# pangfumin/badslam

Hardware: AMD Instinct MI355X
Metric: surfel x keyframe residual evaluations per second, full alternating BA iteration (higher is better)
Workload: dtype f32

## Files before the change

### badslam_amd/abi.py

```python
import ctypes as C

BSLAM_INVALID_DEPTH_BIT = 1 << 15
BSLAM_UNKNOWN_DEPTH = 65535
BSLAM_SURFEL_ACTIVE_FLAG = 1

SURFEL_X, SURFEL_Y, SURFEL_Z, SURFEL_NORMAL = 0, 1, 2, 3
SURFEL_RADIUS_SQUARED, SURFEL_COLOR, SURFEL_DESCRIPTOR1, SURFEL_DESCRIPTOR2 = 4, 5, 6, 7
SURFEL_ACCUM0 = 8
SURFEL_DATA_ATTRIBUTE_COUNT = 8
SURFEL_ATTRIBUTE_COUNT = 17

KF_ACTIVE, KF_COVISIBLE_ACTIVE, KF_INACTIVE = 0, 1, 2

TEX_FIXED_POINT_1_8 = 0
TEX_EXACT_FLOAT = 1

INVALID_INDEX = 0xFFFFFFFF


class Buffer2D(C.Structure):
    _fields_ = [("address", C.c_void_p), ("height", C.c_int32), ("width", C.c_int32), ("pitch", C.c_size_t)]


class Mat3x4(C.Structure):
# ... 138 lines not shown
    "bslam_compute_cost_and_residual_count_from_images": (C.c_int, [C.c_void_p, C.c_void_p, C.c_int, C.c_int, P(Camera4f), P(Camera4f), C.c_float,
                                                                   C.c_float, P(Buffer2D), P(Buffer2D), P(Buffer2D), P(Mat3x4), P(Buffer2D),
                                                                   P(Buffer2D), P(Buffer2D), P(C.c_uint32), P(C.c_float)]),
    "bslam_accumulate_pose_coeffs_from_images_gradmag": (C.c_int, [C.c_void_p, C.c_void_p, C.c_int, C.c_int, P(Camera4f), P(Camera4f), C.c_float, C.c_float,
                                                                  P(Buffer2D), P(Buffer2D), P(Buffer2D), P(Mat3x4), P(Buffer2D), P(Buffer2D), P(Buffer2D),
                                                                  P(C.c_uint32), P(C.c_float), P(C.c_float)]),
    "bslam_compute_cost_and_residual_count_from_images_gradmag": (C.c_int, [C.c_void_p, C.c_void_p, C.c_int, C.c_int, P(Camera4f), P(Camera4f), C.c_float,
                                                                           C.c_float, P(Buffer2D), P(Buffer2D), P(Buffer2D), P(Mat3x4), P(Buffer2D),
                                                                           P(Buffer2D), P(Buffer2D), P(C.c_uint32), P(C.c_float)]),
    "bslam_accumulate_pose_coeffs_from_images_batched": (C.c_int, [C.c_void_p, C.c_void_p, C.c_int, C.c_int, P(Camera4f), P(Camera4f), C.c_float,
                                                                  C.c_float, C.c_int, P(Buffer2D), P(Buffer2D), P(Buffer2D), P(Mat3x4), P(Buffer2D),
                                                                  P(Buffer2D), P(Buffer2D), P(C.c_uint32), P(C.c_float), P(C.c_float)]),
    "bslam_compute_sobel_gradient_magnitude": (C.c_int, [C.c_void_p, C.c_void_p, P(Buffer2D), P(Buffer2D)]),
    "bslam_calibrate_and_downsample_images": (C.c_int, [C.c_void_p, C.c_void_p, C.c_int, P(DepthParams), P(Buffer2D), P(Buffer2D), P(Buffer2D), P(Buffer2D),
                                                       P(Buffer2D), P(Buffer2D)]),
    "bslam_compact_surfels": (C.c_int, [C.c_void_p, C.c_void_p, C.c_uint32, P(C.c_uint32), P(Buffer2D), P(Buffer2D)]),
    "bslam_invalidate_keyframe_cache": (C.c_int, [C.c_void_p]),
    "bslam_comm_get_unique_id": (C.c_int, [C.c_void_p, C.c_size_t]),
    "bslam_comm_init": (C.c_int, [C.c_void_p, C.c_void_p, C.c_int, C.c_int]),
    "bslam_comm_destroy": (C.c_int, [C.c_void_p]),
    "bslam_comm_query": (C.c_int, [C.c_void_p, P(C.c_int), P(C.c_int)]),
    "bslam_set_culling": (C.c_int, [C.c_void_p, C.c_int]),
    "bslam_set_pose_keyframe_list": (C.c_int, [C.c_void_p, C.c_int]),
    "bslam_debug_cull_stats": (C.c_int, [C.c_void_p, P(C.c_uint64), P(C.c_uint64)]),
    "bslam_profile_enable": (C.c_int, [C.c_void_p, C.c_int]),
    "bslam_profile_read": (C.c_int, [C.c_void_p, C.c_int, P(C.c_int32), P(C.c_float)]),
    "bslam_profile_read_counters": (C.c_int, [C.c_void_p, P(C.c_uint64)]),
    "bslam_set_geometry_keyframe_chunk": (C.c_int, [C.c_void_p, C.c_int]),
    "bslam_assign_colors": (C.c_int, [C.c_void_p, C.c_void_p, _CAM, _CAM, _DP, C.c_int, _KFS, C.c_uint32, _BUF]),
    "bslam_debug_decode_normals": (C.c_int, [C.c_void_p, C.c_void_p, P(C.c_float)]),
    "bslam_debug_jacobians": (C.c_int, [C.c_void_p, C.c_void_p, C.c_int, C.c_int, P(C.c_float), P(C.c_float)]),
    "bslam_debug_wave_column_sums": (C.c_int, [C.c_void_p, C.c_void_p, C.c_int, C.c_int, C.POINTER(C.c_float), C.POINTER(C.c_float)]),
    "bslam_debug_desc_pair": (C.c_int, [C.c_void_p, C.c_void_p, C.c_int, P(C.c_float), P(C.c_float)]),
    "bslam_debug_quad_samples": (C.c_int, [C.c_void_p, C.c_void_p, C.c_int, C.c_int, C.c_int, C.c_int, P(C.c_uint8), C.c_int, P(C.c_float), C.c_int,
                                           P(C.c_float), P(C.c_uint16)]),
    "bslam_debug_count_pairs": (C.c_int, [
        C.c_void_p, C.c_void_p, _CAM, _DP, C.c_int, _KFS, C.c_uint32, _BUF, P(C.c_uint64), P(C.c_uint64)]),
    "bslam_accumulate_pose_estimation_coeffs": (C.c_int, [
        C.c_void_p, C.c_void_p, C.c_int, C.c_int, _CAM, _CAM, _DP, _BUF, _BUF, _BUF, P(Mat3x4),
        C.c_uint32, _BUF, C.c_int, P(C.c_uint32), P(C.c_float), P(C.c_float), P(C.c_float)]),
    "bslam_estimate_frame_poses_batched": (C.c_int, [
        C.c_void_p, C.c_void_p, C.c_int, C.c_int, _CAM, _CAM, _DP, C.c_int, _KFS,
        C.c_uint32, _BUF, C.c_int, P(SE3f), P(C.c_int32), P(C.c_int32), ALLREDUCE_FN, C.c_void_p]),
    "bslam_compute_ba_cost": (C.c_int, [
        C.c_void_p, C.c_void_p, C.c_int, C.c_int, _CAM, _CAM, _DP, C.c_int, _KFS,
        C.c_uint32, _BUF, _BUF, P(C.c_float), P(C.c_uint32), ALLREDUCE_FN, C.c_void_p]),
# ... 31 lines not shown
```

### badslam_amd/csrc/badslam_hip.hip

```cpp
#include <hip/hip_runtime.h>
#include <dlfcn.h>
#include <rocprim/device/device_radix_sort.hpp>

#include <algorithm>
#include <climits>
#include <cmath>
#include <cstdlib>
#include <cstring>
#include <initializer_list>
#include <new>

#include "context.hpp"
#include "geometry_kernels.hpp"
#include "intrinsics_kernels.hpp"
#include "pcg_kernels.hpp"
#include "lifecycle_kernels.hpp"
#include "preprocess_kernels.hpp"
#include "rectify_kernels.hpp"
#include "render_kernels.hpp"
#include "fusion_kernels.hpp"
#include "mesh_kernels.hpp"
#include "distance_kernels.hpp"
#include "registration_kernels.hpp"
#include "sampling_kernels.hpp"
#include "simplify_kernels.hpp"
#include "decimate_kernels.hpp"
#include "smooth_kernels.hpp"
#include "raycast_kernels.hpp"
#include "render_mesh_kernels.hpp"
#include "place_kernels.hpp"
#include "odometry_kernels.hpp"
#include "pose_kernels.hpp"
#include "cost_kernels.hpp"
// ... 421 lines not shown
  if (chunks < 1) chunks = 1;
  if (chunks > kf_count) chunks = kf_count;
  int per_block = (kf_count + chunks - 1) / chunks;
#ifndef BSLAM_POSE_MAX_KFS_PER_BLOCK
#define BSLAM_POSE_MAX_KFS_PER_BLOCK 0
#endif
  const int cap = BSLAM_POSE_MAX_KFS_PER_BLOCK > 0 ? BSLAM_POSE_MAX_KFS_PER_BLOCK : (tiles >= 8192 ? 64 : 32);
  per_block = (per_block + multiple - 1) / multiple * multiple;
  if (per_block > cap) per_block = cap;
  return per_block;
}

static unsigned long long* cull_stats_ptr(bslam_context* ctx) {
  return ctx->profiling ? (unsigned long long*)((uint8_t*)ctx->misc.ptr + kMiscCullStats) : nullptr;
}

struct PoseGrid {
  Schedule sc;
  int per_block;
  unsigned chunks;
  unsigned launch_chunks;
  dim3 grid;
};
static int plan_pose_grid(bslam_context* ctx, const Schedule& prepared, int kf_count, int multiple, int list_bound, PoseGrid* g) {
  g->sc = prepared;
#ifndef BSLAM_POSE_CULL_MIN_KEYFRAMES
#define BSLAM_POSE_CULL_MIN_KEYFRAMES 64
#endif
  if (kf_count < BSLAM_POSE_CULL_MIN_KEYFRAMES) g->sc.bounds = nullptr;
  g->per_block = choose_kfs_per_block((int)g->sc.slots, kf_count, multiple);
  g->chunks = (unsigned)((kf_count + g->per_block - 1) / g->per_block);
  g->launch_chunks = list_bound >= 0 ? (unsigned)std::max(1, (std::min(list_bound, kf_count) + g->per_block - 1) / g->per_block) : g->chunks;
  g->grid = dim3(8u * g->sc.slots_per_xcd * g->launch_chunks);
  return ctx->vis.reserve((size_t)g->chunks * g->sc.slots * sizeof(VisWord));
}

static int launch_pose_accumulate(bslam_context* ctx, hipStream_t stream, int use_depth, int use_desc, const CamConsts& c,
                                  int kf_count, uint32_t surfels_size, const bslam_buffer2d* surfels, const PoseState* states,
                                  int* tiles_out, bool reduce_rows = true, const SurfelWork* work = nullptr, int* kfs_per_block_out = nullptr,
                                  bool want_cost = false, const int* kf_list = nullptr, int kf_list_bound = 0) {
  SurfelWork local;
  int rc = BSLAM_OK;
  if (!work) {
    if ((rc = prepare_surfels(ctx, stream, surfels, surfels_size, pose_surfels_per_thread(use_desc != 0, surfels_size), kf_count, &local, use_desc != 0))) return rc;
    work = &local;
  }
  const int tiles = (int)work->sc.slots;
  *tiles_out = tiles;
  const int rows_per_kf = tiles;
  rc = ctx->partials.reserve((size_t)rows_per_kf * kf_count * kRow * sizeof(float));
  if (rc) return rc;
  rc = ctx->coeffs.reserve((size_t)kf_count * kRow * sizeof(float));
  if (rc) return rc;
#ifndef BSLAM_POSE_DESC_KF_MULTIPLE
#define BSLAM_POSE_DESC_KF_MULTIPLE 4
#endif
  PoseGrid g;
  if ((rc = plan_pose_grid(ctx, work->sc, kf_count, use_desc ? BSLAM_POSE_DESC_KF_MULTIPLE : 1, kf_list ? kf_list_bound : -1, &g))) return rc;
  const Schedule& sc = g.sc;
  const int per_block = g.per_block;
  if (kfs_per_block_out) *kfs_per_block_out = per_block;
  VisWord* vis = (VisWord*)ctx->vis.ptr;
  const dim3 grid = g.grid;
  const SurfelRows rows = work->rows;
  const KfDev* kfs = (const KfDev*)ctx->kf_table.ptr;
  float* partials = (float*)ctx->partials.ptr;
  static const unsigned debug_lds = getenv("BSLAM_DEBUG_POSE_LDS") ? (unsigned)atoi(getenv("BSLAM_DEBUG_POSE_LDS")) : 0u;
  {
  ProfScope prof(ctx, stream);
  const bool cost = want_cost;
#define BSLAM_LAUNCH_POSE(DEPTH, DESC, R)                                                                                                        \
  do {                                                                                                                                           \
    if (cost) hipLaunchKernelGGL((pose_accumulate_kernel<DEPTH, DESC, R, true>), grid, dim3(kPoseThreads), debug_lds, stream, c, kfs, kf_count, per_block, sc, rows, partials, rows_per_kf, states, vis, kf_list);  \
    else hipLaunchKernelGGL((pose_accumulate_kernel<DEPTH, DESC, R, false>), grid, dim3(kPoseThreads), debug_lds, stream, c, kfs, kf_count, per_block, sc, rows, partials, rows_per_kf, states, vis, kf_list); \
  } while (0)
  if (use_depth && use_desc) BSLAM_LAUNCH_POSE(true, true, kPoseRDesc);
  else if (use_depth && pose_surfels_per_thread(false, surfels_size) == kPoseRGeoLarge) BSLAM_LAUNCH_POSE(true, false, kPoseRGeoLarge);
  else if (use_depth) BSLAM_LAUNCH_POSE(true, false, kPoseRGeo);
  else BSLAM_LAUNCH_POSE(false, true, kPoseRDesc);
#undef BSLAM_LAUNCH_POSE
  }
  BSLAM_HIP_TRY(hipGetLastError());
  if (!reduce_rows) return BSLAM_OK;
  hipLaunchKernelGGL(pose_reduce_rows_kernel, dim3((unsigned)kf_count), dim3(1024), (unsigned)visit_map_bytes(tiles), stream, (const float*)partials, rows_per_kf, kf_count,
                     (float*)ctx->coeffs.ptr, states, (const VisWord*)vis, per_block, cull_stats_ptr(ctx), kf_list ? kf_list + 1 + kf_count : nullptr);
// ... 177 lines not shown
}

int bslam_set_xcd_schedule(bslam_context* ctx, int enable) {
  if (!ctx) return fail(BSLAM_ERR_INVALID_ARGUMENT, "context is null");
  ctx->use_schedule = enable != 0;
  ctx->order_key.clear();
  ctx->perm_key.clear();
  return BSLAM_OK;
}

int bslam_set_culling(bslam_context* ctx, int enable) {
  if (!ctx) return fail(BSLAM_ERR_INVALID_ARGUMENT, "context is null");
  ctx->culling = enable != 0;
  return BSLAM_OK;
}

int bslam_set_pose_keyframe_list(bslam_context* ctx, int min_keyframes) {
  if (!ctx) return fail(BSLAM_ERR_INVALID_ARGUMENT, "null context");
  if (min_keyframes < 0) return fail(BSLAM_ERR_INVALID_ARGUMENT, "min_keyframes must be >= 0");
  ctx->pose_list_min_keyframes = min_keyframes;
  return BSLAM_OK;
}

int bslam_debug_cull_stats(bslam_context* ctx, uint64_t* tested, uint64_t* culled) {
  if (!ctx) return fail(BSLAM_ERR_INVALID_ARGUMENT, "context is null");
  BSLAM_HIP_TRY(hipSetDevice(ctx->device));
  BSLAM_HIP_TRY(hipDeviceSynchronize());
  unsigned long long h[2] = {0, 0};
  BSLAM_HIP_TRY(hipMemcpy(h, (uint8_t*)ctx->misc.ptr + kMiscCullStats, sizeof(h), hipMemcpyDeviceToHost));
  BSLAM_HIP_TRY(hipMemset((uint8_t*)ctx->misc.ptr + kMiscCullStats, 0, sizeof(h)));
  if (tested) *tested = h[0];
  if (culled) *culled = h[0] - h[1];
  return BSLAM_OK;
}

int bslam_profile_enable(bslam_context* ctx, int enable) {
  if (!ctx) return fail(BSLAM_ERR_INVALID_ARGUMENT, "context is null");
  ctx->profiling = enable != 0;
  for (auto& ev : ctx->prof_pending) ctx->prof_pool.push_back(std::make_pair(ev.start, ev.stop));
  ctx->prof_pending.clear();
  for (int t = 0; t < 8; ++t) { ctx->prof_launches[t] = 0; ctx->prof_ms[t] = 0.f; }
  for (int i = 0; i < 8; ++i) ctx->prof_counter_base[i] = 0;
  if (ctx->prof_counters.ptr && ctx->prof_counter_slots) {
    BSLAM_HIP_TRY(hipSetDevice(ctx->device));
    BSLAM_HIP_TRY(hipDeviceSynchronize());
    BSLAM_HIP_TRY(hipMemset(ctx->prof_counters.ptr, 0, ctx->prof_counter_slots * sizeof(unsigned long long)));
// ... 282 lines not shown
  if (rc) return rc;
  std::vector<PoseState> states((size_t)keyframe_count);
  for (int k = 0; k < keyframe_count; ++k) {
    PoseState& st = states[k];
    std::memset(&st, 0, sizeof(st));
    std::memcpy(st.q, poses[k].q, sizeof(float) * 4);
    std::memcpy(st.t, poses[k].t, sizeof(float) * 3);
    st.converged = (keyframes[k].activation == BSLAM_KF_INACTIVE) ? 1 : 0;
  }
  const size_t state_bytes = states.size() * sizeof(PoseState);
  if ((rc = ctx->pose_state.reserve(state_bytes))) return rc;
  if ((rc = ctx->staging2.reserve(state_bytes + 64))) return rc;
  {
    void* stage = nullptr;
    if ((rc = ctx->upload_ring.acquire(state_bytes, &stage))) return rc;
    std::memcpy(stage, states.data(), state_bytes);
    BSLAM_HIP_TRY(hipMemcpyAsync(ctx->pose_state.ptr, stage, state_bytes, hipMemcpyHostToDevice, stream));
    if ((rc = ctx->upload_ring.commit(stream))) return rc;
  }

  PoseState* d_states = (PoseState*)ctx->pose_state.ptr;
  int* d_active = (int*)((uint8_t*)ctx->misc.ptr + kMiscActive);
  int* h_active = (int*)((uint8_t*)ctx->staging2.ptr + state_bytes);
  for (hipEvent_t& e : ctx->iter_done)
    if (!e) BSLAM_HIP_TRY(hipEventCreateWithFlags(&e, hipEventDisableTiming));
  for (hipEvent_t& e : ctx->solve_done)
    if (!e) BSLAM_HIP_TRY(hipEventCreateWithFlags(&e, hipEventDisableTiming));
  if (!ctx->copy_stream) BSLAM_HIP_TRY(hipStreamCreateWithFlags(&ctx->copy_stream, hipStreamNonBlocking));
  ctx->kf_table_host_ptr = nullptr;
  hipLaunchKernelGGL(pose_init_kernel, dim3((unsigned)((keyframe_count + 63) / 64)), dim3(64), 0, stream, keyframe_count,
                     (const PoseState*)d_states, (KfDev*)ctx->kf_table.ptr, d_active);
  BSLAM_HIP_TRY(hipGetLastError());

  SurfelWork work;
  if (surfels_size > 0 && (rc = prepare_surfels(ctx, stream, surfels, surfels_size, pose_surfels_per_thread(use_descriptor_residuals != 0, surfels_size), keyframe_count, &work, use_descriptor_residuals != 0))) return rc;

  int* d_list = nullptr;
  if (surfels_size > 0 && ctx->pose_list_min_keyframes > 0 && keyframe_count >= ctx->pose_list_min_keyframes) {
    if ((rc = ctx->pose_list.reserve((size_t)(1 + 2 * keyframe_count) * sizeof(int)))) return rc;
    d_list = (int*)ctx->pose_list.ptr;
    hipLaunchKernelGGL(pose_active_list_kernel, dim3(1), dim3(kActiveListThreads), 0, stream, keyframe_count, (const PoseState*)d_states, d_list);
    BSLAM_HIP_TRY(hipGetLastError());
  }
  int known_active = keyframe_count;

  auto enqueue_iteration = [&](int it) -> int {
    const int slot = it & 3;
    const bool exchange = allreduce != nullptr || has_exchange(ctx);
    const bool fused = surfels_size > 0 && !exchange;
    if (fused) {
      int tiles = 0, per_block = 1;
      int r = launch_pose_accumulate(ctx, stream, use_depth_residuals, use_descriptor_residuals, c, keyframe_count, surfels_size, surfels, d_states, &tiles, false, &work, &per_block,
                                     false, d_list, known_active);
      if (r) return r;
      {
        ProfScope prof(ctx, stream, BSLAM_PROF_POSE_REDUCE);
        hipLaunchKernelGGL(pose_reduce_solve_kernel, dim3((unsigned)keyframe_count), dim3(kReduceSolveThreads), (unsigned)visit_map_bytes(tiles), stream, (const float*)ctx->partials.ptr,
                           tiles, keyframe_count, d_states, (KfDev*)ctx->kf_table.ptr, d_active + slot, d_active + ((it + 1) & 3),
                           (const VisWord*)ctx->vis.ptr, per_block, cull_stats_ptr(ctx), d_list ? d_list + 1 + keyframe_count : nullptr);
      }
      BSLAM_HIP_TRY(hipGetLastError());
    } else {
      if (surfels_size > 0) {
        int tiles = 0;
        int r = launch_pose_accumulate(ctx, stream, use_depth_residuals, use_descriptor_residuals, c, keyframe_count, surfels_size, surfels, d_states, &tiles, true, &work, nullptr,
                                       false, d_list, known_active);
        if (r) return r;
      } else {
        int r = ctx->coeffs.reserve((size_t)keyframe_count * kRow * sizeof(float));
        if (r) return r;
        BSLAM_HIP_TRY(hipMemsetAsync(ctx->coeffs.ptr, 0, (size_t)keyframe_count * kRow * sizeof(float), stream));
      }
      {
        ProfScope prof(ctx, stream, BSLAM_PROF_EXCHANGE);
        if (allreduce) {
          const int arc = allreduce(allreduce_user, ctx->coeffs.ptr, (size_t)keyframe_count * kRow, stream);
          if (arc) return fail(BSLAM_ERR_HIP, "allreduce callback failed with %d", arc);
        } else if (exchange) {
          const int arc = exchange_sum(ctx, stream, (float*)ctx->coeffs.ptr, (size_t)keyframe_count * kRow);
          if (arc) return arc;
        }
      }
      hipLaunchKernelGGL(pose_solve_kernel, dim3((unsigned)((keyframe_count + 63) / 64)), dim3(64), 0, stream,
                         (const float*)ctx->coeffs.ptr, keyframe_count, d_states, (KfDev*)ctx->kf_table.ptr, d_active + slot, d_active + ((it + 1) & 3));
      BSLAM_HIP_TRY(hipGetLastError());
    }
    BSLAM_HIP_TRY(hipEventRecord(ctx->solve_done[slot], stream));
    BSLAM_HIP_TRY(hipStreamWaitEvent(ctx->copy_stream, ctx->solve_done[slot], 0));
    BSLAM_HIP_TRY(hipMemcpyAsync(h_active + slot, d_active + slot, sizeof(int), hipMemcpyDeviceToHost, ctx->copy_stream));
    BSLAM_HIP_TRY(hipEventRecord(ctx->iter_done[slot], ctx->copy_stream));
    if (d_list) {
      hipLaunchKernelGGL(pose_active_list_kernel, dim3(1), dim3(kActiveListThreads), 0, stream, keyframe_count, (const PoseState*)d_states, d_list);
      BSLAM_HIP_TRY(hipGetLastError());
    }
    return BSLAM_OK;
  };
  if (max_iterations > 0 && (rc = enqueue_iteration(0))) return rc;
  for (int it = 0; it < max_iterations; ++it) {
    if (it + 1 < max_iterations && (rc = enqueue_iteration(it + 1))) return rc;
    BSLAM_HIP_TRY(hipEventSynchronize(ctx->iter_done[it & 3]));
    if (h_active[it & 3] == 0) break;
    known_active = std::min(known_active, h_active[it & 3]);
  }
  BSLAM_HIP_TRY(hipMemcpyAsync(ctx->staging2.ptr, d_states, state_bytes, hipMemcpyDeviceToHost, stream));
  BSLAM_HIP_TRY(hipStreamSynchronize(stream));
  BSLAM_HIP_TRY(hipStreamSynchronize(ctx->copy_stream));
  const PoseState* out = (const PoseState*)ctx->staging2.ptr;
  for (int k = 0; k < keyframe_count; ++k) {
    std::memcpy(poses[k].q, out[k].q, sizeof(float) * 4);
    std::memcpy(poses[k].t, out[k].t, sizeof(float) * 3);
    if (iterations_done) iterations_done[k] = out[k].iterations;
    if (converged) converged[k] = (keyframes[k].activation == BSLAM_KF_INACTIVE) ? 1 : out[k].converged;
  }
  return BSLAM_OK;
}


int bslam_update_surfel_activation(
    bslam_context* ctx, void* stream_, const bslam_camera4f* depth_camera, const bslam_depth_params* depth_params,
    int keyframe_count, const bslam_keyframe_view* keyframes, uint32_t surfels_size, const bslam_buffer2d* surfels,
    const bslam_buffer2d* active_surfels) {
  hipStream_t stream = (hipStream_t)stream_;
  if (surfels_size == 0) return BSLAM_OK;
  if (!active_surfels) return fail(BSLAM_ERR_INVALID_ARGUMENT, "active_surfels is null");
  CamConsts c;
// ... 166 lines not shown
```

### badslam_amd/csrc/context.hpp

```cpp
#pragma once

#include <hip/hip_runtime.h>

#include <cstdarg>
#include <cstdio>
#include <string>
#include <vector>

#include "device_math.hpp"

namespace bslam {

extern thread_local std::string g_last_error;

inline int fail(int code, const char* fmt, ...) {
  char buf[512];
  va_list ap;
  va_start(ap, fmt);
  vsnprintf(buf, sizeof(buf), fmt, ap);
  va_end(ap);
  g_last_error = buf;
  return code;
}

#define BSLAM_HIP_TRY(expr)                                                                         \
  do {                                                                                              \
    hipError_t e_ = (expr);                                                                         \
    if (e_ != hipSuccess) return ::bslam::fail(BSLAM_ERR_HIP, "%s failed: %s", #expr, hipGetErrorString(e_)); \
  } while (0)

constexpr size_t kMiscActive = 0;
constexpr size_t kMiscPairCensus = 64;
constexpr size_t kMiscPcgScratch = 128;
constexpr size_t kMiscPcgPair = 160;
constexpr size_t kMiscDeleted = 192;
constexpr size_t kMiscMinMaxDepth = 208;
constexpr size_t kMiscCullStats = 224;
constexpr size_t kMiscBytes = 256;

template <bool kPinned>
struct GrowingSlab {
  void* ptr = nullptr;
  size_t bytes = 0;
  GrowingSlab() = default;
  GrowingSlab(const GrowingSlab&) = delete;
  GrowingSlab& operator=(const GrowingSlab&) = delete;
  ~GrowingSlab() { release(); }
  int reserve(size_t need) {
    if (need <= bytes) return BSLAM_OK;
    release();
    const size_t want = need + need / 4 + 256;
    const hipError_t e = kPinned ? hipHostMalloc(&ptr, want, hipHostMallocDefault) : hipMalloc(&ptr, want);
    if (e != hipSuccess) {
// ... 78 lines not shown
    return BSLAM_OK;
  }
};

}

struct bslam_context {
  int device = 0;
  int tex_mode = BSLAM_TEX_FIXED_POINT_1_8;
  int cu_count = 256;
  bslam::Slab kf_table;
  bslam::Slab records;
  bslam::Slab quads;
  bslam::Slab partials;
  bslam::Slab coeffs;
  bslam::Slab pose_state;
  bslam::Slab misc;
  bslam::Slab intr_cells;
  int geom_kf_chunk = -1;
  int intr_cells_owner = 0;
  size_t intr_cells_cells = 0;
  bslam::PinnedSlab staging2;
  bslam::StagingRing upload_ring;
  hipEvent_t iter_done[4] = {};
  hipEvent_t solve_done[4] = {};
  hipStream_t copy_stream = nullptr;
  std::vector<uint8_t> kf_table_host;
  const void* kf_table_host_ptr = nullptr;
  bool keyframe_cache = false;
  std::vector<uint64_t> records_signature;
  std::vector<uint64_t> quads_signature;
  bslam::Slab quads_aux;
  bslam::Slab lifecycle;
  bslam::Slab zbuffer;
  int render_mesh_small_box = 64, render_mesh_wave_box = 256;
  bool render_mesh_project_once = false, render_mesh_resolve_projected = false;
  bslam::Slab place_pattern;
  bool place_pattern_ready = false;
  bslam::Slab fusion;
  bslam::Slab distance;
  bslam::Slab registration;
  struct PreparedMesh {
    bool ready = false;
    float radius = 0.f;
    float origin[3] = {0.f, 0.f, 0.f}, inv_cell = 0.f;
    int dim[3] = {0, 0, 0};
    uint32_t cells = 0, valid = 0, triangles = 0;
    void *records = nullptr, *cell_count = nullptr, *cell_start = nullptr, *list = nullptr;
  } prepared;
// ... 22 lines not shown
  int sorted_key_rows = 0;
  bool sorted_key_bounds = false;
  uint64_t sorted_key_perm_serial = 0;
  uint64_t perm_serial = 0;
  bslam::Slab pose_list;
  bslam::Slab vis;
  bool culling = true;
  int pose_list_min_keyframes = 64;
  bslam::SurfelKey perm_key;
  hipEvent_t perm_ready = nullptr;
  hipStream_t perm_stream = nullptr;
  bool use_schedule = true;
  bslam::SurfelKey order_key;
  bool profiling = false;
  struct ProfEntry { hipEvent_t start, stop; int tag; };
  std::vector<ProfEntry> prof_pending;
  std::vector<std::pair<hipEvent_t, hipEvent_t>> prof_pool;
  int prof_launches[8] = {0, 0, 0, 0, 0, 0, 0, 0};
  float prof_ms[8] = {0.f, 0.f, 0.f, 0.f, 0.f, 0.f, 0.f, 0.f};
  bslam::Slab prof_counters;
  size_t prof_counter_slots = 0;
  uint64_t prof_counter_base[8] = {0, 0, 0, 0, 0, 0, 0, 0};
  ~bslam_context() {
    for (hipEvent_t e : iter_done) if (e) { hipError_t err = hipEventDestroy(e); (void)err; }
    for (hipEvent_t e : solve_done) if (e) { hipError_t err = hipEventDestroy(e); (void)err; }
    if (perm_ready) { hipError_t err = hipEventDestroy(perm_ready); (void)err; }
    if (copy_stream) { hipError_t err = hipStreamDestroy(copy_stream); (void)err; }
    for (const ProfEntry& p : prof_pending) { hipError_t err = hipEventDestroy(p.start); err = hipEventDestroy(p.stop); (void)err; }
    for (const auto& p : prof_pool) { hipError_t err = hipEventDestroy(p.first); err = hipEventDestroy(p.second); (void)err; }
  }
};

namespace bslam {
int rccl_allreduce_sum(bslam_context* ctx, hipStream_t stream, float* device_buffer, size_t count);
inline bool has_exchange(const bslam_context* ctx) { return ctx->allreduce != nullptr || ctx->comm != nullptr; }
inline int exchange_sum(bslam_context* ctx, hipStream_t stream, float* device_buffer, size_t count) {
  if (ctx->allreduce) {
    const int arc = ctx->allreduce(ctx->allreduce_user, device_buffer, count, stream);
    if (arc) return fail(BSLAM_ERR_HIP, "allreduce callback failed with %d", arc);
    return BSLAM_OK;
  }
  if (ctx->comm) return rccl_allreduce_sum(ctx, stream, device_buffer, count);
  return BSLAM_OK;
}

struct ProfScope {
  bslam_context* ctx; hipStream_t stream; std::pair<hipEvent_t, hipEvent_t> ev; bool on; int tag;
  ProfScope(bslam_context* c, hipStream_t s, int tag_ = 0) : ctx(c), stream(s), on(c->profiling), tag(tag_) {
// ... 13 lines not shown
```

### badslam_amd/csrc/pose_kernels.hpp

```cpp
#pragma once

#include "device_math.hpp"

namespace bslam {

constexpr int kPoseThreads = 256;
#ifndef BSLAM_POSE_R_GEO
#define BSLAM_POSE_R_GEO 4
#endif
#ifndef BSLAM_POSE_R_DESC
#define BSLAM_POSE_R_DESC 2
#endif
constexpr int kPoseRGeo = BSLAM_POSE_R_GEO;
constexpr int kPoseRDesc = BSLAM_POSE_R_DESC;
#ifndef BSLAM_POSE_R_GEO_LARGE
#define BSLAM_POSE_R_GEO_LARGE 6
#endif
constexpr int kPoseRGeoLarge = BSLAM_POSE_R_GEO_LARGE;
constexpr uint32_t kPoseLargeSurfels = 2000000u;
inline int pose_surfels_per_thread(bool use_desc, uint32_t surfels_size) {
  return use_desc ? kPoseRDesc : (surfels_size >= kPoseLargeSurfels ? kPoseRGeoLarge : kPoseRGeo);
}
constexpr int kRow = 32;
constexpr int kRowCost = 27;
// ... 560 lines not shown
    for (int i = k + 1; i < n; ++i)
      if (perm[k] == i) swap_d(y[k], y[i]);
  }
#pragma unroll
  for (int i = 0; i < n; ++i)
#pragma unroll
    for (int j = 0; j < i; ++j) y[i] -= A[i][j] * y[j];
#pragma unroll
  for (int i = 0; i < n; ++i) { const double d = A[i][i]; y[i] = (fabs(d) > 2.2250738585072014e-308) ? y[i] / d : 0.0; }
#pragma unroll
  for (int i = n - 1; i >= 0; --i)
#pragma unroll
    for (int j = i + 1; j < n; ++j) y[i] -= A[j][i] * y[j];
#pragma unroll
  for (int k = n - 1; k >= 0; --k) {
#pragma unroll
    for (int i = k + 1; i < n; ++i)
      if (perm[k] == i) swap_d(y[k], y[i]);
  }
#pragma unroll
  for (int i = 0; i < n; ++i) x[i] = (float)y[i];
}

__global__ void pose_init_kernel(int kf_count, const PoseState* __restrict__ states, KfDev* __restrict__ kfs, int* __restrict__ active_counters) {
  const int k = blockIdx.x * blockDim.x + threadIdx.x;
  if (k < 4) active_counters[k] = 0;
  if (k >= kf_count) return;
  const PoseState st = states[k];
  se3_inverse_matrix(Quat{st.q[0], st.q[1], st.q[2], st.q[3]}, mk3(st.t[0], st.t[1], st.t[2]), kfs[k].frame_T_global.m);
}

constexpr int kActiveListThreads = 1024;
__global__ __launch_bounds__(kActiveListThreads) void pose_active_list_kernel(int kf_count, const PoseState* __restrict__ states, int* __restrict__ out) {
  __shared__ int wave_total[kActiveListThreads / 64];
  __shared__ int base;
  int* list = out + 1;
  int* pos = out + 1 + kf_count;
  const int lane = threadIdx.x & 63, wave = threadIdx.x >> 6;
  if (threadIdx.x == 0) base = 0;
  __syncthreads();
  for (int k0 = 0; k0 < kf_count; k0 += kActiveListThreads) {
    const int k = k0 + (int)threadIdx.x;
    const bool active = k < kf_count && !states[k].converged;
    const unsigned long long mask = __ballot(active);
    if (lane == 0) wave_total[wave] = __builtin_popcountll(mask);
    __syncthreads();
    int before = base;
    for (int w = 0; w < wave; ++w) before += wave_total[w];
    if (active) {
      const int place = before + __builtin_popcountll(mask & ((1ull << lane) - 1ull));
      list[place] = k;
      pos[k] = place;
    } else if (k < kf_count) {
      pos[k] = -1;
    }
    __syncthreads();
    if (threadIdx.x == 0) {
      int t = base;
      for (int w = 0; w < kActiveListThreads / 64; ++w) t += wave_total[w];
      base = t;
    }
    __syncthreads();
  }
  if (threadIdx.x == 0) out[0] = base;
}

__device__ __forceinline__ void pose_update(int k, PoseState st, const float* H, const float* b, PoseState* __restrict__ states,
                                            KfDev* __restrict__ kfs, int* __restrict__ active_count) {
  float x[6];
  solve_ldlt6(H, b, x);
  float neg[6];
  for (int i = 0; i < 6; ++i) neg[i] = -1.f * x[i];
  Quat dq; f3 dt;
  se3_exp(neg, &dq, &dt);
  Quat q{st.q[0], st.q[1], st.q[2], st.q[3]};
  f3 t = mk3(st.t[0], st.t[1], st.t[2]);
// ... 4 lines not shown
  st.q[0] = q.x; st.q[1] = q.y; st.q[2] = q.z; st.q[3] = q.w;
  st.t[0] = t.x; st.t[1] = t.y; st.t[2] = t.z;
  st.iterations += 1;
  st.converged = (nrm < 1e-06f) ? 1 : 0;
  states[k] = st;
  se3_inverse_matrix(q, t, kfs[k].frame_T_global.m);
  if (!st.converged) atomicAdd(active_count, 1);
}

__global__ void pose_solve_kernel(const float* __restrict__ coeffs, int kf_count, PoseState* __restrict__ states,
                                  KfDev* __restrict__ kfs, int* __restrict__ active_count, int* __restrict__ next_active_count) {
  const int k = blockIdx.x * blockDim.x + threadIdx.x;
  if (k == 0 && next_active_count != nullptr) *next_active_count = 0;
  if (k >= kf_count) return;
  const PoseState st = states[k];
  if (st.converged) return;
  float H[21], b[6];
  for (int i = 0; i < 21; ++i) H[i] = coeffs[(size_t)k * kRow + i];
  for (int i = 0; i < 6; ++i) b[i] = coeffs[(size_t)k * kRow + 21 + i];
  pose_update(k, st, H, b, states, kfs, active_count);
}

constexpr int kReduceSolveThreads = 1024;
__global__ __launch_bounds__(kReduceSolveThreads) void pose_reduce_solve_kernel(const float* __restrict__ partials, int rows_per_kf, int kf_count,
                                                                               PoseState* __restrict__ states, KfDev* __restrict__ kfs,
                                                                               int* __restrict__ active_count, int* __restrict__ next_active_count,
                                                                               const VisWord* __restrict__ vis, int kfs_per_block, unsigned long long* __restrict__ stats,
                                                                               const int* __restrict__ kf_pos) {
  const int k = blockIdx.x;
  if (k == 0 && threadIdx.x == 0) *next_active_count = 0;
  if (states[k].converged) return;
  __shared__ float sm[32][kRow];
  __shared__ float row[kRow];
  pose_sum_rows(partials, rows_per_kf, k, vis, kfs_per_block, stats, kf_pos, sm);
  if (threadIdx.x < 27) {
    float total = 0.f;
    for (int i = 0; i < 32; ++i) total += sm[i][threadIdx.x];
    row[threadIdx.x] = total;
  }
  __syncthreads();
  if (threadIdx.x != 0) return;
  float H[21], b[6];
  for (int i = 0; i < 21; ++i) H[i] = row[i];
  for (int i = 0; i < 6; ++i) b[i] = row[21 + i];
  pose_update(k, states[k], H, b, states, kfs, active_count);
}

}
```

### include/badslam_hip.h

```cpp
#ifndef BADSLAM_HIP_H_
#define BADSLAM_HIP_H_

#include <stddef.h>
#include <stdint.h>

#ifdef __cplusplus
extern "C" {
#endif


enum {
  BSLAM_INVALID_DEPTH_BIT = 1 << 15,
  BSLAM_UNKNOWN_DEPTH = 65535,
  BSLAM_SURFEL_ACTIVE_FLAG = 1,

  BSLAM_SURFEL_X = 0,
  BSLAM_SURFEL_Y = 1,
  BSLAM_SURFEL_Z = 2,
  BSLAM_SURFEL_NORMAL = 3,
  BSLAM_SURFEL_RADIUS_SQUARED = 4,
  BSLAM_SURFEL_COLOR = 5,
  BSLAM_SURFEL_DESCRIPTOR1 = 6,
  BSLAM_SURFEL_DESCRIPTOR2 = 7,
  BSLAM_SURFEL_ACCUM0 = 8,
// ... 72 lines not shown
  BSLAM_TEX_FIXED_POINT_1_8 = 0,
  BSLAM_TEX_EXACT_FLOAT = 1
};

typedef struct bslam_context bslam_context;


int bslam_abi_version(void);

const char* bslam_last_error(void);

int bslam_create(int device, bslam_context** out_ctx);
int bslam_destroy(bslam_context* ctx);

int bslam_set_texture_mode(bslam_context* ctx, int mode);

int bslam_set_keyframe_cache(bslam_context* ctx, int enable);
int bslam_invalidate_keyframe_cache(bslam_context* ctx);

int bslam_set_xcd_schedule(bslam_context* ctx, int enable);

int bslam_set_culling(bslam_context* ctx, int enable);
int bslam_set_pose_keyframe_list(bslam_context* ctx, int min_keyframes);
int bslam_debug_cull_stats(bslam_context* ctx, uint64_t* tested, uint64_t* culled);

int bslam_profile_enable(bslam_context* ctx, int enable);
enum { BSLAM_PROF_POSE_ACCUMULATE = 0, BSLAM_PROF_GEOMETRY = 1, BSLAM_PROF_PCG_INIT = 2, BSLAM_PROF_PCG_STEP1 = 3, BSLAM_PROF_ACTIVATION = 4,
       BSLAM_PROF_EXCHANGE = 5,
       BSLAM_PROF_POSE_REDUCE = 6,
       BSLAM_PROF_BA_COST = 7 };
int bslam_profile_read(bslam_context* ctx, int kernel, int32_t* launches, float* total_ms);
int bslam_profile_read_counters(bslam_context* ctx, uint64_t* counters8);


int bslam_accumulate_pose_estimation_coeffs(
    bslam_context* ctx, void* stream,
    int use_depth_residuals, int use_descriptor_residuals,
    const bslam_camera4f* color_camera, const bslam_camera4f* depth_camera,
    const bslam_depth_params* depth_params,
    const bslam_buffer2d* depth_buffer, const bslam_buffer2d* normals_buffer,
    const bslam_buffer2d* color_buffer,
    const bslam_mat3x4* frame_T_global_estimate,
    uint32_t surfels_size, const bslam_buffer2d* surfels,
    int debug, uint32_t* residual_count, float* residual_sum,
    float* H, float* b);

// ... 417 lines not shown
```

Baseline: 194.8 billion.

## Split pose estimation into keyframe groups on separate streams with independent convergence

```diff
diff --git a/badslam_amd/abi.py b/badslam_amd/abi.py
--- a/badslam_amd/abi.py
+++ b/badslam_amd/abi.py
@@ -184,6 +184,7 @@
     "bslam_comm_query": (C.c_int, [C.c_void_p, P(C.c_int), P(C.c_int)]),
     "bslam_set_culling": (C.c_int, [C.c_void_p, C.c_int]),
     "bslam_set_pose_keyframe_list": (C.c_int, [C.c_void_p, C.c_int]),
+    "bslam_set_pose_keyframe_groups": (C.c_int, [C.c_void_p, C.c_int, C.c_int]),
     "bslam_debug_cull_stats": (C.c_int, [C.c_void_p, P(C.c_uint64), P(C.c_uint64)]),
     "bslam_profile_enable": (C.c_int, [C.c_void_p, C.c_int]),
     "bslam_profile_read": (C.c_int, [C.c_void_p, C.c_int, P(C.c_int32), P(C.c_float)]),
diff --git a/badslam_amd/csrc/badslam_hip.hip b/badslam_amd/csrc/badslam_hip.hip
--- a/badslam_amd/csrc/badslam_hip.hip
+++ b/badslam_amd/csrc/badslam_hip.hip
@@ -9,6 +9,7 @@
 #include <cstring>
 #include <initializer_list>
 #include <new>
+#include <thread>
 
 #include "context.hpp"
 #include "geometry_kernels.hpp"
@@ -476,7 +477,7 @@
   unsigned launch_chunks;
   dim3 grid;
 };
-static int plan_pose_grid(bslam_context* ctx, const Schedule& prepared, int kf_count, int multiple, int list_bound, PoseGrid* g) {
+static int plan_pose_grid(bslam_context* ctx, const Schedule& prepared, int kf_count, int multiple, int list_bound, PoseGrid* g, int range_count = -1) {
   g->sc = prepared;
 #ifndef BSLAM_POSE_CULL_MIN_KEYFRAMES
 #define BSLAM_POSE_CULL_MIN_KEYFRAMES 64
@@ -484,15 +485,22 @@
   if (kf_count < BSLAM_POSE_CULL_MIN_KEYFRAMES) g->sc.bounds = nullptr;
   g->per_block = choose_kfs_per_block((int)g->sc.slots, kf_count, multiple);
   g->chunks = (unsigned)((kf_count + g->per_block - 1) / g->per_block);
-  g->launch_chunks = list_bound >= 0 ? (unsigned)std::max(1, (std::min(list_bound, kf_count) + g->per_block - 1) / g->per_block) : g->chunks;
+  g->launch_chunks = list_bound >= 0 ? (unsigned)std::max(1, (std::min(list_bound, range_count >= 0 ? range_count : kf_count) + g->per_block - 1) / g->per_block) : g->chunks;
   g->grid = dim3(8u * g->sc.slots_per_xcd * g->launch_chunks);
   return ctx->vis.reserve((size_t)g->chunks * g->sc.slots * sizeof(VisWord));
+}
+
+#ifndef BSLAM_POSE_DESC_KF_MULTIPLE
+#define BSLAM_POSE_DESC_KF_MULTIPLE 4
+#endif
+static VisWord* range_vis(bslam_context* ctx, int first, int per_block, int slots) {
+  return (VisWord*)ctx->vis.ptr + (size_t)(first / per_block) * slots;
 }
 
 static int launch_pose_accumulate(bslam_context* ctx, hipStream_t stream, int use_depth, int use_desc, const CamConsts& c,
                                   int kf_count, uint32_t surfels_size, const bslam_buffer2d* surfels, const PoseState* states,
                                   int* tiles_out, bool reduce_rows = true, const SurfelWork* work = nullptr, int* kfs_per_block_out = nullptr,
-                                  bool want_cost = false, const int* kf_list = nullptr, int kf_list_bound = 0) {
+                                  bool want_cost = false, const int* kf_list = nullptr, int kf_list_bound = 0, int range_first = 0, int range_count = -1) {
   SurfelWork local;
   int rc = BSLAM_OK;
   if (!work) {
@@ -506,15 +514,12 @@
   if (rc) return rc;
   rc = ctx->coeffs.reserve((size_t)kf_count * kRow * sizeof(float));
   if (rc) return rc;
-#ifndef BSLAM_POSE_DESC_KF_MULTIPLE
-#define BSLAM_POSE_DESC_KF_MULTIPLE 4
-#endif
   PoseGrid g;
-  if ((rc = plan_pose_grid(ctx, work->sc, kf_count, use_desc ? BSLAM_POSE_DESC_KF_MULTIPLE : 1, kf_list ? kf_list_bound : -1, &g))) return rc;
+  if ((rc = plan_pose_grid(ctx, work->sc, kf_count, use_desc ? BSLAM_POSE_DESC_KF_MULTIPLE : 1, kf_list ? kf_list_bound : -1, &g, range_count))) return rc;
   const Schedule& sc = g.sc;
   const int per_block = g.per_block;
   if (kfs_per_block_out) *kfs_per_block_out = per_block;
-  VisWord* vis = (VisWord*)ctx->vis.ptr;
+  VisWord* vis = range_vis(ctx, range_first, per_block, tiles);
   const dim3 grid = g.grid;
   const SurfelRows rows = work->rows;
   const KfDev* kfs = (const KfDev*)ctx->kf_table.ptr;
@@ -738,6 +743,15 @@
   return BSLAM_OK;
 }
 
+int bslam_set_pose_keyframe_groups(bslam_context* ctx, int groups, int min_keyframes_per_group) {
+  if (!ctx) return fail(BSLAM_ERR_INVALID_ARGUMENT, "null context");
+  if (groups < 0 || groups > bslam::kMaxPoseGroups) return fail(BSLAM_ERR_INVALID_ARGUMENT, "groups must be 0 (default) .. %d", bslam::kMaxPoseGroups);
+  if (min_keyframes_per_group < 0) return fail(BSLAM_ERR_INVALID_ARGUMENT, "min_keyframes_per_group must be >= 0");
+  ctx->pose_groups = groups;
+  ctx->pose_group_min_keyframes = min_keyframes_per_group;
+  return BSLAM_OK;
+}
+
 int bslam_debug_cull_stats(bslam_context* ctx, uint64_t* tested, uint64_t* culled) {
   if (!ctx) return fail(BSLAM_ERR_INVALID_ARGUMENT, "context is null");
   BSLAM_HIP_TRY(hipSetDevice(ctx->device));
@@ -1066,85 +1080,159 @@
   PoseState* d_states = (PoseState*)ctx->pose_state.ptr;
   int* d_active = (int*)((uint8_t*)ctx->misc.ptr + kMiscActive);
   int* h_active = (int*)((uint8_t*)ctx->staging2.ptr + state_bytes);
-  for (hipEvent_t& e : ctx->iter_done)
-    if (!e) BSLAM_HIP_TRY(hipEventCreateWithFlags(&e, hipEventDisableTiming));
-  for (hipEvent_t& e : ctx->solve_done)
-    if (!e) BSLAM_HIP_TRY(hipEventCreateWithFlags(&e, hipEventDisableTiming));
+  static_assert(kMaxPoseGroups * 4 * sizeof(int) <= 64 && kMiscActive + kMaxPoseGroups * 4 * sizeof(int) <= kMiscPairCensus, "room for every group's counters");
   if (!ctx->copy_stream) BSLAM_HIP_TRY(hipStreamCreateWithFlags(&ctx->copy_stream, hipStreamNonBlocking));
   ctx->kf_table_host_ptr = nullptr;
   hipLaunchKernelGGL(pose_init_kernel, dim3((unsigned)((keyframe_count + 63) / 64)), dim3(64), 0, stream, keyframe_count,
-                     (const PoseState*)d_states, (KfDev*)ctx->kf_table.ptr, d_active);
+                     (const PoseState*)d_states, (KfDev*)ctx->kf_table.ptr, d_active, kMaxPoseGroups * 4);
   BSLAM_HIP_TRY(hipGetLastError());
 
   SurfelWork work;
   if (surfels_size > 0 && (rc = prepare_surfels(ctx, stream, surfels, surfels_size, pose_surfels_per_thread(use_descriptor_residuals != 0, surfels_size), keyframe_count, &work, use_descriptor_residuals != 0))) return rc;
 
-  int* d_list = nullptr;
-  if (surfels_size > 0 && ctx->pose_list_min_keyframes > 0 && keyframe_count >= ctx->pose_list_min_keyframes) {
-    if ((rc = ctx->pose_list.reserve((size_t)(1 + 2 * keyframe_count) * sizeof(int)))) return rc;
-    d_list = (int*)ctx->pose_list.ptr;
-    hipLaunchKernelGGL(pose_active_list_kernel, dim3(1), dim3(kActiveListThreads), 0, stream, keyframe_count, (const PoseState*)d_states, d_list);
-    BSLAM_HIP_TRY(hipGetLastError());
-  }
-  int known_active = keyframe_count;
-
-  auto enqueue_iteration = [&](int it) -> int {
+  const bool use_list = surfels_size > 0 && ctx->pose_list_min_keyframes > 0 && keyframe_count >= ctx->pose_list_min_keyframes;
+  const bool exchange = allreduce != nullptr || has_exchange(ctx);
+  const bool fused = surfels_size > 0 && !exchange;
+
+#ifndef BSLAM_POSE_GROUPS_DEFAULT
+#define BSLAM_POSE_GROUPS_DEFAULT 1
+#endif
+#ifndef BSLAM_POSE_GROUP_MIN_KEYFRAMES
+#define BSLAM_POSE_GROUP_MIN_KEYFRAMES 64
+#endif
+  struct Group {
+    int first, count;
+    hipStream_t stream;
+    int* d_list;
+    int known_active;
+    bool live;
+  };
+  Group groups[kMaxPoseGroups];
+  const int chunk_len = surfels_size > 0 ? choose_kfs_per_block((int)work.sc.slots, keyframe_count, use_descriptor_residuals ? BSLAM_POSE_DESC_KF_MULTIPLE : 1) : 1;
+  const int chunk_count = (keyframe_count + chunk_len - 1) / chunk_len;
+  int G = 1;
+  if (fused && use_list) {
+    G = ctx->pose_groups > 0 ? ctx->pose_groups : BSLAM_POSE_GROUPS_DEFAULT;
+    const int min_per_group = ctx->pose_group_min_keyframes > 0 ? ctx->pose_group_min_keyframes : BSLAM_POSE_GROUP_MIN_KEYFRAMES;
+    G = std::max(1, std::min(std::min(G, kMaxPoseGroups), std::min(keyframe_count / min_per_group, chunk_count)));
+  }
+  int* d_pos = nullptr;
+  if (use_list) {
+    if ((rc = ctx->pose_list.reserve((size_t)(2 * keyframe_count + G) * sizeof(int)))) return rc;
+    d_pos = (int*)ctx->pose_list.ptr + keyframe_count + G;
+  }
+  for (int g = 0; g < G; ++g) {
+    Group& gr = groups[g];
+    gr.first = (int)((long long)chunk_count * g / G) * chunk_len;
+    gr.count = (g + 1 == G ? keyframe_count : (int)((long long)chunk_count * (g + 1) / G) * chunk_len) - gr.first;
+    gr.known_active = gr.count;
+    gr.live = true;
+    gr.d_list = use_list ? (int*)ctx->pose_list.ptr + gr.first + g : nullptr;
+    if (g > 0 && !ctx->group_stream[g]) BSLAM_HIP_TRY(hipStreamCreateWithFlags(&ctx->group_stream[g], hipStreamNonBlocking));
+    gr.stream = g == 0 ? stream : ctx->group_stream[g];
+    for (hipEvent_t* e : {&ctx->iter_done[g][0], &ctx->iter_done[g][1], &ctx->iter_done[g][2], &ctx->iter_done[g][3], &ctx->solve_done[g][0], &ctx->solve_done[g][1],
+                          &ctx->solve_done[g][2], &ctx->solve_done[g][3], &ctx->group_first[g], &ctx->group_end[g]})
+      if (!*e) BSLAM_HIP_TRY(hipEventCreateWithFlags(e, hipEventDisableTiming));
+  }
+  if (G > 1) {
+    if (!ctx->group_fork) BSLAM_HIP_TRY(hipEventCreateWithFlags(&ctx->group_fork, hipEventDisableTiming));
+    BSLAM_HIP_TRY(hipEventRecord(ctx->group_fork, stream));
+    for (int g = 1; g < G; ++g) BSLAM_HIP_TRY(hipStreamWaitEvent(groups[g].stream, ctx->group_fork, 0));
+  }
+  if (use_list)
+    for (int g = 0; g < G; ++g) {
+      hipLaunchKernelGGL(pose_active_list_kernel, dim3(1), dim3(kActiveListThreads), 0, groups[g].stream, groups[g].first, groups[g].count, (const PoseState*)d_states,
+                         groups[g].d_list, d_pos);
+      BSLAM_HIP_TRY(hipGetLastError());
+    }
+
+  auto enqueue_iteration = [&](int g, int it) -> int {
+    const Group& gr = groups[g];
+    hipStream_t gs = gr.stream;
     const int slot = it & 3;
-    const bool exchange = allreduce != nullptr || has_exchange(ctx);
-    const bool fused = surfels_size > 0 && !exchange;
+    int* active = d_active + 4 * g;
     if (fused) {
+      if (it == 0 && g > 0) BSLAM_HIP_TRY(hipStreamWaitEvent(gs, ctx->group_first[g - 1], 0));
       int tiles = 0, per_block = 1;
-      int r = launch_pose_accumulate(ctx, stream, use_depth_residuals, use_descriptor_residuals, c, keyframe_count, surfels_size, surfels, d_states, &tiles, false, &work, &per_block,
-                                     false, d_list, known_active);
+      int r = launch_pose_accumulate(ctx, gs, use_depth_residuals, use_descriptor_residuals, c, keyframe_count, surfels_size, surfels, d_states, &tiles, false, &work, &per_block,
+                                     false, gr.d_list, gr.known_active, gr.first, gr.count);
       if (r) return r;
+      if (it == 0 && g + 1 < G) BSLAM_HIP_TRY(hipEventRecord(ctx->group_first[g], gs));
       {
-        ProfScope prof(ctx, stream, BSLAM_PROF_POSE_REDUCE);
-        hipLaunchKernelGGL(pose_reduce_solve_kernel, dim3((unsigned)keyframe_count), dim3(kReduceSolveThreads), (unsigned)visit_map_bytes(tiles), stream, (const float*)ctx->partials.ptr,
-                           tiles, keyframe_count, d_states, (KfDev*)ctx->kf_table.ptr, d_active + slot, d_active + ((it + 1) & 3),
-                           (const VisWord*)ctx->vis.ptr, per_block, cull_stats_ptr(ctx), d_list ? d_list + 1 + keyframe_count : nullptr);
+        ProfScope prof(ctx, gs, BSLAM_PROF_POSE_REDUCE);
+        hipLaunchKernelGGL(pose_reduce_solve_kernel, dim3((unsigned)gr.count), dim3(kReduceSolveThreads), (unsigned)visit_map_bytes(tiles), gs, (const float*)ctx->partials.ptr,
+                           tiles, gr.first, d_states, (KfDev*)ctx->kf_table.ptr, active + slot, active + ((it + 1) & 3),
+                           (const VisWord*)range_vis(ctx, gr.first, per_block, tiles), per_block, cull_stats_ptr(ctx), (const int*)d_pos);
       }
       BSLAM_HIP_TRY(hipGetLastError());
     } else {
       if (surfels_size > 0) {
         int tiles = 0;
-        int r = launch_pose_accumulate(ctx, stream, use_depth_residuals, use_descriptor_residuals, c, keyframe_count, surfels_size, surfels, d_states, &tiles, true, &work, nullptr,
-                                       false, d_list, known_active);
+        int r = launch_pose_accumulate(ctx, gs, use_depth_residuals, use_descriptor_residuals, c, keyframe_count, surfels_size, surfels, d_states, &tiles, true, &work, nullptr,
+                                       false, gr.d_list, gr.known_active);
         if (r) return r;
       } else {
         int r = ctx->coeffs.reserve((size_t)keyframe_count * kRow * sizeof(float));
         if (r) return r;
-        BSLAM_HIP_TRY(hipMemsetAsync(ctx->coeffs.ptr, 0, (size_t)keyframe_count * kRow * sizeof(float), stream));
+        BSLAM_HIP_TRY(hipMemsetAsync(ctx->coeffs.ptr, 0, (size_t)keyframe_count * kRow * sizeof(float), gs));
       }
       {
-        ProfScope prof(ctx, stream, BSLAM_PROF_EXCHANGE);
+        ProfScope prof(ctx, gs, BSLAM_PROF_EXCHANGE);
         if (allreduce) {
-          const int arc = allreduce(allreduce_user, ctx->coeffs.ptr, (size_t)keyframe_count * kRow, stream);
+          const int arc = allreduce(allreduce_user, ctx->coeffs.ptr, (size_t)keyframe_count * kRow, gs);
           if (arc) return fail(BSLAM_ERR_HIP, "allreduce callback failed with %d", arc);
         } else if (exchange) {
-          const int arc = exchange_sum(ctx, stream, (float*)ctx->coeffs.ptr, (size_t)keyframe_count * kRow);
+          const int arc = exchange_sum(ctx, gs, (float*)ctx->coeffs.ptr, (size_t)keyframe_count * kRow);
           if (arc) return arc;
         }
       }
-      hipLaunchKernelGGL(pose_solve_kernel, dim3((unsigned)((keyframe_count + 63) / 64)), dim3(64), 0, stream,
-                         (const float*)ctx->coeffs.ptr, keyframe_count, d_states, (KfDev*)ctx->kf_table.ptr, d_active + slot, d_active + ((it + 1) & 3));
+      hipLaunchKernelGGL(pose_solve_kernel, dim3((unsigned)((keyframe_count + 63) / 64)), dim3(64), 0, gs,
+                         (const float*)ctx->coeffs.ptr, keyframe_count, d_states, (KfDev*)ctx->kf_table.ptr, active + slot, active + ((it + 1) & 3));
       BSLAM_HIP_TRY(hipGetLastError());
     }
-    BSLAM_HIP_TRY(hipEventRecord(ctx->solve_done[slot], stream));
-    BSLAM_HIP_TRY(hipStreamWaitEvent(ctx->copy_stream, ctx->solve_done[slot], 0));
-    BSLAM_HIP_TRY(hipMemcpyAsync(h_active + slot, d_active + slot, sizeof(int), hipMemcpyDeviceToHost, ctx->copy_stream));
-    BSLAM_HIP_TRY(hipEventRecord(ctx->iter_done[slot], ctx->copy_stream));
-    if (d_list) {
-      hipLaunchKernelGGL(pose_active_list_kernel, dim3(1), dim3(kActiveListThreads), 0, stream, keyframe_count, (const PoseState*)d_states, d_list);
+    hipStream_t flag_stream = G > 1 ? gs : ctx->copy_stream;
+    if (G == 1) {
+      BSLAM_HIP_TRY(hipEventRecord(ctx->solve_done[g][slot], gs));
+      BSLAM_HIP_TRY(hipStreamWaitEvent(flag_stream, ctx->solve_done[g][slot], 0));
+    }
+    BSLAM_HIP_TRY(hipMemcpyAsync(h_active + 4 * g + slot, active + slot, sizeof(int), hipMemcpyDeviceToHost, flag_stream));
+    BSLAM_HIP_TRY(hipEventRecord(ctx->iter_done[g][slot], flag_stream));
+    if (gr.d_list) {
+      hipLaunchKernelGGL(pose_active_list_kernel, dim3(1), dim3(kActiveListThreads), 0, gs, gr.first, gr.count, (const PoseState*)d_states, gr.d_list, d_pos);
       BSLAM_HIP_TRY(hipGetLastError());
     }
     return BSLAM_OK;
   };
-  if (max_iterations > 0 && (rc = enqueue_iteration(0))) return rc;
-  for (int it = 0; it < max_iterations; ++it) {
-    if (it + 1 < max_iterations && (rc = enqueue_iteration(it + 1))) return rc;
-    BSLAM_HIP_TRY(hipEventSynchronize(ctx->iter_done[it & 3]));
-    if (h_active[it & 3] == 0) break;
-    known_active = std::min(known_active, h_active[it & 3]);
+  int waits_for[kMaxPoseGroups] = {0, 0, 0, 0};
+  int live = max_iterations > 0 ? G : 0;
+  for (int it = 0; it < 2 && it < max_iterations; ++it)
+    for (int g = 0; g < G; ++g)
+      if ((rc = enqueue_iteration(g, it))) return rc;
+  while (live > 0) {
+    bool progressed = false;
+    for (int g = 0; g < G; ++g) {
+      Group& gr = groups[g];
+      if (!gr.live) continue;
+      const int it = waits_for[g];
+      if (live > 1) {
+        const hipError_t q = hipEventQuery(ctx->iter_done[g][it & 3]);
+        if (q == hipErrorNotReady) { (void)hipGetLastError(); continue; }
+        if (q != hipSuccess) return fail(BSLAM_ERR_HIP, "hipEventQuery failed: %s", hipGetErrorString(q));
+      } else {
+        BSLAM_HIP_TRY(hipEventSynchronize(ctx->iter_done[g][it & 3]));
+      }
+      progressed = true;
+      const int left = h_active[4 * g + (it & 3)];
+      waits_for[g] = it + 1;
+      if (left == 0 || it + 1 >= max_iterations) { gr.live = false; --live; continue; }
+      gr.known_active = std::min(gr.known_active, left);
+      if (it + 2 < max_iterations && (rc = enqueue_iteration(g, it + 2))) return rc;
+    }
+    if (!progressed) std::this_thread::yield();
+  }
+  for (int g = 1; g < G; ++g) {
+    BSLAM_HIP_TRY(hipEventRecord(ctx->group_end[g], groups[g].stream));
+    BSLAM_HIP_TRY(hipStreamWaitEvent(stream, ctx->group_end[g], 0));
   }
   BSLAM_HIP_TRY(hipMemcpyAsync(ctx->staging2.ptr, d_states, state_bytes, hipMemcpyDeviceToHost, stream));
   BSLAM_HIP_TRY(hipStreamSynchronize(stream));
diff --git a/badslam_amd/csrc/context.hpp b/badslam_amd/csrc/context.hpp
--- a/badslam_amd/csrc/context.hpp
+++ b/badslam_amd/csrc/context.hpp
@@ -29,6 +29,7 @@
     if (e_ != hipSuccess) return ::bslam::fail(BSLAM_ERR_HIP, "%s failed: %s", #expr, hipGetErrorString(e_)); \
   } while (0)
 
+constexpr int kMaxPoseGroups = 4;
 constexpr size_t kMiscActive = 0;
 constexpr size_t kMiscPairCensus = 64;
 constexpr size_t kMiscPcgScratch = 128;
@@ -153,9 +154,15 @@
   size_t intr_cells_cells = 0;
   bslam::PinnedSlab staging2;
   bslam::StagingRing upload_ring;
-  hipEvent_t iter_done[4] = {};
-  hipEvent_t solve_done[4] = {};
+  hipEvent_t iter_done[bslam::kMaxPoseGroups][4] = {};
+  hipEvent_t solve_done[bslam::kMaxPoseGroups][4] = {};
   hipStream_t copy_stream = nullptr;
+  hipStream_t group_stream[bslam::kMaxPoseGroups] = {};
+  hipEvent_t group_fork = nullptr;
+  hipEvent_t group_first[bslam::kMaxPoseGroups] = {};
+  hipEvent_t group_end[bslam::kMaxPoseGroups] = {};
+  int pose_groups = 0;
+  int pose_group_min_keyframes = 0;
   std::vector<uint8_t> kf_table_host;
   const void* kf_table_host_ptr = nullptr;
   bool keyframe_cache = false;
@@ -224,8 +231,14 @@
   size_t prof_counter_slots = 0;
   uint64_t prof_counter_base[8] = {0, 0, 0, 0, 0, 0, 0, 0};
   ~bslam_context() {
-    for (hipEvent_t e : iter_done) if (e) { hipError_t err = hipEventDestroy(e); (void)err; }
-    for (hipEvent_t e : solve_done) if (e) { hipError_t err = hipEventDestroy(e); (void)err; }
+    for (int g = 0; g < bslam::kMaxPoseGroups; ++g) {
+      for (hipEvent_t e : iter_done[g]) if (e) { hipError_t err = hipEventDestroy(e); (void)err; }
+      for (hipEvent_t e : solve_done[g]) if (e) { hipError_t err = hipEventDestroy(e); (void)err; }
+      if (group_first[g]) { hipError_t err = hipEventDestroy(group_first[g]); (void)err; }
+      if (group_end[g]) { hipError_t err = hipEventDestroy(group_end[g]); (void)err; }
+      if (group_stream[g]) { hipError_t err = hipStreamDestroy(group_stream[g]); (void)err; }
+    }
+    if (group_fork) { hipError_t err = hipEventDestroy(group_fork); (void)err; }
     if (perm_ready) { hipError_t err = hipEventDestroy(perm_ready); (void)err; }
     if (copy_stream) { hipError_t err = hipStreamDestroy(copy_stream); (void)err; }
     for (const ProfEntry& p : prof_pending) { hipError_t err = hipEventDestroy(p.start); err = hipEventDestroy(p.stop); (void)err; }
diff --git a/badslam_amd/csrc/pose_kernels.hpp b/badslam_amd/csrc/pose_kernels.hpp
--- a/badslam_amd/csrc/pose_kernels.hpp
+++ b/badslam_amd/csrc/pose_kernels.hpp
@@ -606,26 +606,28 @@
   for (int i = 0; i < n; ++i) x[i] = (float)y[i];
 }
 
-__global__ void pose_init_kernel(int kf_count, const PoseState* __restrict__ states, KfDev* __restrict__ kfs, int* __restrict__ active_counters) {
+__global__ void pose_init_kernel(int kf_count, const PoseState* __restrict__ states, KfDev* __restrict__ kfs, int* __restrict__ active_counters,
+                                 int counter_count) {
   const int k = blockIdx.x * blockDim.x + threadIdx.x;
-  if (k < 4) active_counters[k] = 0;
+  if (k < counter_count) active_counters[k] = 0;
   if (k >= kf_count) return;
   const PoseState st = states[k];
   se3_inverse_matrix(Quat{st.q[0], st.q[1], st.q[2], st.q[3]}, mk3(st.t[0], st.t[1], st.t[2]), kfs[k].frame_T_global.m);
 }
 
 constexpr int kActiveListThreads = 1024;
-__global__ __launch_bounds__(kActiveListThreads) void pose_active_list_kernel(int kf_count, const PoseState* __restrict__ states, int* __restrict__ out) {
+__global__ __launch_bounds__(kActiveListThreads) void pose_active_list_kernel(int kf_first, int kf_count, const PoseState* __restrict__ states, int* __restrict__ out,
+                                                                              int* __restrict__ pos) {
   __shared__ int wave_total[kActiveListThreads / 64];
   __shared__ int base;
   int* list = out + 1;
-  int* pos = out + 1 + kf_count;
   const int lane = threadIdx.x & 63, wave = threadIdx.x >> 6;
+  const int kf_end = kf_first + kf_count;
   if (threadIdx.x == 0) base = 0;
   __syncthreads();
-  for (int k0 = 0; k0 < kf_count; k0 += kActiveListThreads) {
+  for (int k0 = kf_first; k0 < kf_end; k0 += kActiveListThreads) {
     const int k = k0 + (int)threadIdx.x;
-    const bool active = k < kf_count && !states[k].converged;
+    const bool active = k < kf_end && !states[k].converged;
     const unsigned long long mask = __ballot(active);
     if (lane == 0) wave_total[wave] = __builtin_popcountll(mask);
     __syncthreads();
@@ -635,7 +637,7 @@
       const int place = before + __builtin_popcountll(mask & ((1ull << lane) - 1ull));
       list[place] = k;
       pos[k] = place;
-    } else if (k < kf_count) {
+    } else if (k < kf_end) {
       pos[k] = -1;
     }
     __syncthreads();
@@ -686,13 +688,13 @@
 }
 
 constexpr int kReduceSolveThreads = 1024;
-__global__ __launch_bounds__(kReduceSolveThreads) void pose_reduce_solve_kernel(const float* __restrict__ partials, int rows_per_kf, int kf_count,
+__global__ __launch_bounds__(kReduceSolveThreads) void pose_reduce_solve_kernel(const float* __restrict__ partials, int rows_per_kf, int kf_first,
                                                                                PoseState* __restrict__ states, KfDev* __restrict__ kfs,
                                                                                int* __restrict__ active_count, int* __restrict__ next_active_count,
                                                                                const VisWord* __restrict__ vis, int kfs_per_block, unsigned long long* __restrict__ stats,
                                                                                const int* __restrict__ kf_pos) {
-  const int k = blockIdx.x;
-  if (k == 0 && threadIdx.x == 0) *next_active_count = 0;
+  const int k = kf_first + (int)blockIdx.x;
+  if (blockIdx.x == 0 && threadIdx.x == 0) *next_active_count = 0;
   if (states[k].converged) return;
   __shared__ float sm[32][kRow];
   __shared__ float row[kRow];
diff --git a/include/badslam_hip.h b/include/badslam_hip.h
--- a/include/badslam_hip.h
+++ b/include/badslam_hip.h
@@ -118,6 +118,7 @@
 
 int bslam_set_culling(bslam_context* ctx, int enable);
 int bslam_set_pose_keyframe_list(bslam_context* ctx, int min_keyframes);
+int bslam_set_pose_keyframe_groups(bslam_context* ctx, int groups, int min_keyframes_per_group);
 int bslam_debug_cull_stats(bslam_context* ctx, uint64_t* tested, uint64_t* culled);
 
 int bslam_profile_enable(bslam_context* ctx, int enable);
```

Result: no change. 194.9 billion (median of 3 runs) (+0.0%).
